# kamalmostafa/minimodem

Hardware: AMD Instinct MI355X
Metric: audio samples/sec demodulated (whole node), 1200-baud 48 kHz f32 (higher is better)
Workload: dtype f64; 1 GPU; configs[1]: Bell202 1200-baud, 48 kHz f32, batch of 1024 synthetic streams; 1024 streams x 480000 samples per GPU (BASELINE.json); streams_per_gpu=1024, total_streams=1024, input_dtype=f32, accumulate_dtype=f64

## Files before the change

minimodem_amd/__init__.py:

```python
import contextlib
import ctypes as C
import os
import subprocess

import numpy as np

from . import _lib
from ._lib import ModemArgs, RxConfig

__all__ = ["build", "rx_config", "Context", "demod_batch", "find_frame_batch",
           "LegacyPlan", "synthesize", "FRAME_DTYPE", "EPISODE_DTYPE",
           "gather_bytes", "shard_range"]

_HERE = os.path.dirname(os.path.abspath(__file__))

FRAME_DTYPE = np.dtype([("bits", "<u8"), ("start", "<u8"), ("confidence", "<f4"),
                        ("amplitude", "<f4"), ("flags", "<u4"), ("reserved", "<u4")])
EPISODE_DTYPE = np.dtype([("carrier_nsamples", "<u8"), ("first_frame", "<u4"),
                          ("nframes", "<u4"), ("confidence_total", "<f4"),
                          ("amplitude_total", "<f4"), ("end_reason", "<u4"),
                          ("b_mark", "<u4")])
SEARCH_DTYPE = np.dtype([("sample_offset", "<u8"), ("navail", "<u4"), ("try_first", "<u4"),
                         ("try_max", "<u4"), ("try_step", "<u4"), ("search_limit", "<f4"),
                         ("use_sync_string", "<u4")])
RESULT_DTYPE = np.dtype([("bits", "<u8"), ("confidence", "<f4"), ("amplitude", "<f4"),
                         ("frame_start", "<u4"), ("n_positions", "<u4")])
assert SEARCH_DTYPE.itemsize == 32 and RESULT_DTYPE.itemsize == 24
NCOUNTERS = 32
COUNTER_NAMES = {0: "iterations", 1: "batches", 2: "stages", 3: "bulk_frames", 4: "refines",
                 5: "cache_hits", 6: "positions", 7: "lattice_batches", 8: "cyc_total",
                 9: "cyc_scan", 10: "cyc_wait", 11: "cyc_confidence", 12: "cyc_bulk", 13: "w_stage", 14: "w_correlate",
                 15: "w_barrier", 16: "cyc_general", 17: "cyc_restart", 18: "cyc_scan1", 19: "cyc_scan2", 20: "cyc_replay_scan", 21: "cyc_scan_wait",
                 24: "conf_fallbacks", 25: "seg_second_looks"}


def build(force=False):
    if force and os.path.exists(_lib.LIB_PATH):
        os.unlink(_lib.LIB_PATH)
    subprocess.run(["make", "-s", "-C", os.path.join(_HERE, "csrc")], check=True)
    return _lib.LIB_PATH


def rx_config(baudmode="1200", **opts):
    lib = _lib.load()
    a = ModemArgs()
    lib.mifsk_modem_args_default(C.byref(a))
    a.baudmode = str(baudmode).encode()
    if "sync_byte" in opts:
        a.have_sync_byte = 1
    for k, v in opts.items():
        if not hasattr(a, k):
            raise TypeError("unknown modem option %r" % k)
        setattr(a, k, v)
    cfg = RxConfig()
    rc = lib.mifsk_rx_config_init(C.byref(cfg), C.byref(a))
    if rc != 0:
        raise ValueError("mifsk_rx_config_init failed: %d" % rc)
    cfg._keepalive = a
    return cfg


class Context:

    def __init__(self, device=-1):
        self._lib = _lib.load()
        h = C.c_void_p()
        rc = self._lib.mifsk_ctx_create(C.byref(h), int(device))
        if rc != 0:
            raise RuntimeError("mifsk_ctx_create failed: %d (no gfx950 HIP device? "
                               "this package has no CPU path)" % rc)
        self.handle = h

    @property
    def device_name(self):
        return self._lib.mifsk_ctx_device_name(self.handle).decode()

    def selftest_sqrt(self, nvalues, seed=1):
        counts = (C.c_uint64 * 4)()
        rc = self._lib.mifsk_selftest_sqrt(self.handle, int(seed), int(nvalues), counts)
        if rc != 0:
            raise RuntimeError("mifsk_selftest_sqrt failed: %d" % rc)
        return tuple(int(c) for c in counts)

    def selftest_rcp(self, c, x):
        c = np.ascontiguousarray(c, np.float32)
        x = np.ascontiguousarray(x, np.float32)
        assert c.shape == x.shape and c.ndim == 1
        rc_out, q = np.empty(c.shape, np.float64), np.empty(c.shape, np.float32)
        rc = self._lib.mifsk_selftest_rcp(self.handle, c.ctypes.data, x.ctypes.data, c.size,
                                          rc_out.ctypes.data, q.ctypes.data)
        if rc != 0:
            raise RuntimeError("mifsk_selftest_rcp failed: %d" % rc)
        return rc_out, q

    def selftest_mag(self, re, im, scalar=1.0):
        re = np.ascontiguousarray(re, np.float64)
        im = np.ascontiguousarray(im, np.float64)
        assert re.shape == im.shape and re.ndim == 1
        root, g = np.empty(re.shape, np.float64), np.empty(re.shape, np.float64)
        unsafe, mag = np.empty(re.shape, np.uint8), np.empty(re.shape, np.float32)
        rc = self._lib.mifsk_selftest_mag(self.handle, re.ctypes.data, im.ctypes.data, float(scalar),
                                          re.size, root.ctypes.data, g.ctypes.data,
                                          unsafe.ctypes.data, mag.ctypes.data)
        if rc != 0:
            raise RuntimeError("mifsk_selftest_mag failed: %d" % rc)
        return root, g, unsafe, mag

    def selftest_confidence(self, variant, mags, req_mask=0, req_val=0):
        mags = np.ascontiguousarray(mags, np.float32)
        assert mags.ndim == 3 and mags.shape[2] == 2
        n = mags.shape[0]
        conf, ampl = np.empty(n, np.float32), np.empty(n, np.float32)
        bits, fb = np.empty(n, np.uint64), np.empty(n, np.uint32)
        rc = self._lib.mifsk_selftest_confidence(self.handle, int(variant), mags.shape[1],
                                                 int(req_mask), int(req_val), mags.ctypes.data, n,
                                                 conf.ctypes.data, ampl.ctypes.data,
# ... 1199 lines not shown
```

minimodem_amd/csrc/mifsk_kernels.hip:

```cpp
#include <hip/hip_runtime.h>
#include <cfloat>
#include <cmath>
#include <cstdint>
#include <cstdlib>
#include <cstdio>
#include <cstring>

#include "mifsk_device.h"
#include "mifsk_devmath.h"
#include "mifsk_devlib.h"
#include "mifsk_rxloop.h"

#ifdef MIFSK_PROFILE
#define MIFSK_CLOCK() ((uint32_t)clock64())
#else
#define MIFSK_CLOCK() 0u
#endif

namespace mifsk {




__global__ __launch_bounds__(64)
// ... 143 lines not shown
	    const uint32_t v = v0 + i * blockDim.x + threadIdx.x;
	    if ( v0 + i * blockDim.x < nvec )
		buf[i] = load4_raw(x, org4 + ( v << 2 ), N);
	}
#pragma unroll
	for ( int i = 0; i < STAGE_VEC; i++ ) {
	    const uint32_t v = v0 + i * blockDim.x + threadIdx.x;
	    if ( v0 + i * blockDim.x < nvec && v < nvec )
		store4_skewed(cfg, lds->slab, slab_cap, v << 2, head, buf[i], org4 + ( v << 2 ), N);
	}
    }
}

template <bool USE_SLAB>
__device__ __forceinline__ void par_correlate( const DevCfg &cfg, const double *__restrict__ tw, StreamLds *lds,
	const float *__restrict__ x, uint32_t N, uint32_t row_org, uint32_t nq )
{
    const uint32_t n_bits = cfg.n_bits;
    const uint32_t B = cfg.bit_nsamples;
    const uint32_t nwin = nq * n_bits;
    for ( uint32_t w0 = 0; w0 < nwin; w0 += blockDim.x ) {
	const uint32_t w = w0 + threadIdx.x;
	if ( w0 + ( threadIdx.x & ~63u ) >= nwin )
	    continue;
	const bool active = w < nwin;
	const uint32_t q = active ? udiv_magic(w, n_bits, cfg.nbits_magic) : 0;
	const uint32_t k = active ? w - q * n_bits : 0;
	const uint32_t a = lds->c_pos[q] + cfg.bit_offset[k];
	double acc[4] = { 0.0, 0.0, 0.0, 0.0 };
	if ( USE_SLAB ) {
	    corr_skewed_stream(cfg, tw, lds->slab, a - row_org, threadIdx.x & 63u, acc);
	} else {
	    for ( uint32_t n = 0; n < B; n++ ) {
		const uint32_t idx = a + n;
		const float xv = ( idx < N && idx >= a ) ? x[idx] : 0.0f;
		const double xd = (double)xv;
		const double *t = tw + 4 * (size_t)n;
		acc[0] = fma(xd, t[0], acc[0]);
		acc[1] = fma(xd, t[1], acc[1]);
		acc[2] = fma(xd, t[2], acc[2]);
		acc[3] = fma(xd, t[3], acc[3]);
	    }
	}
	if ( active )
	    lds->mags[0][w] = band_mag2(acc[0], acc[1], acc[2], acc[3], cfg.magscalar);
    }
}

template <bool USE_SLAB>
__device__ __forceinline__ void scan_part( const DevCfg &cfg, const double *__restrict__ tw,
	StreamLds *lds, const StreamLds::Cmd *cmd, const float *__restrict__ x, uint32_t N,
	uint32_t slab_cap )
{
    const uint32_t nq = cmd->nq;
    const uint32_t row_org = cmd->row_org;
    if ( USE_SLAB && cmd->stage ) {
	par_stage(cfg, lds, x, N, slab_cap, row_org, cmd->stage);
	lds_barrier();
    }
    par_correlate<USE_SLAB>(cfg, tw, lds, x, N, row_org, nq);
    lds_barrier();
}

__device__ __forceinline__ void lds_barrier()
{
    __builtin_amdgcn_fence(__ATOMIC_RELEASE, "workgroup", "local");
    __builtin_amdgcn_s_barrier();
    __builtin_amdgcn_fence(__ATOMIC_ACQUIRE, "workgroup", "local");
}



template <bool USE_SLAB>
struct Master {
    const DevCfg	&cfg;
    const double	*tw;
    const float		*x;
    uint32_t		N;
    StreamLds		*lds;
    uint32_t		slab_cap;
    uint32_t		slab_lo, slab_hi;
    uint32_t		lat_batch;
    uint32_t		conf_idx;
    uint32_t		lat_first;
    uint32_t		spec, run, cold, pause;
    uint32_t		spec_floor;
    uint32_t		lane;
    bool		inflight;
    uint32_t		inflight_anchor, inflight_frames, inflight_buf;
    uint32_t		seq;
    uint32_t		lat_n, lat_anchor;
    uint32_t		hit_base = 0xFFFFFFFFu;
    bool		cnt_on = false;
    uint32_t		cyc_par = 0, cyc_conf = 0, cyc_wait = 0, cyc_scan_wait = 0;
    uint32_t		cyc_sf_load = 0, cyc_sf_corr = 0, cyc_sf_score = 0, cyc_sf_sel = 0;
    uint32_t		h_la, h_la_magic, h_nbits;
    uint64_t		h_req_mask, h_req_val;
    TwGroup		mtg[3];

    template <int NG>
    __device__ __forceinline__ void keep_groups()
    {
#pragma unroll
	for ( int gi = 0; gi < NG; gi++ )
	    mtg[gi] = tw_group_load(tw, (uint32_t)gi, lane);
    }

    __device__ __forceinline__ Master( const DevCfg &c, const double *t, const float *xs,
	    uint32_t n, StreamLds *l, uint32_t cap, uint32_t lf, uint32_t lat_round )
	: cfg(c), tw(t), x(xs), N(n), lds(l), slab_cap(cap), slab_lo(0), slab_hi(0),
	  lat_batch(lf), lane(threadIdx.x), inflight(false), inflight_anchor(0),
	  inflight_frames(0), inflight_buf(0), seq(0), lat_n(0), lat_anchor(0)
    {
	lat_first = lat_round;
	spec = lat_batch;
	run = cold = pause = 0;
	spec_floor = 2;
	h_la = keep_scalar(cfg.lock_advance);
	h_la_magic = keep_scalar(cfg.la_magic);
	h_nbits = keep_scalar(cfg.n_bits);
	h_req_mask = keep_scalar(cfg.req_mask[0]);
	h_req_val = keep_scalar(cfg.req_val[0]);
	conf_idx = lane * cfg.n_bits;
	if ( cfg.lat_grid && lat_round ) {
	    const uint32_t r = lane / lat_round, fr = lane - r * lat_round;
	    conf_idx = r * ( lat_round * ( cfg.n_bits - 1u ) + 1u ) + fr * ( cfg.n_bits - 1u );
	}
    }

    __device__ __forceinline__ void bump( uint32_t which, uint32_t by = 1u ) const
    {
	if ( cnt_on && lane == 0 )
	    (void)__hip_atomic_fetch_add(&lds->cnt[which], by, __ATOMIC_RELAXED, __HIP_MEMORY_SCOPE_WAVEFRONT);
    }

    __device__ __forceinline__ uint32_t lattice_lookup( uint32_t p ) const
    {
	if ( !lat_n || p < lat_anchor )
	    return ~0u;
	const uint32_t d = p - lat_anchor;
	const uint32_t e = udiv_magic(d, h_la, h_la_magic);
	return ( e < lat_n && e * h_la == d ) ? e : ~0u;
    }

    __device__ __forceinline__ StreamLds::Cmd *next_cmd() { return &lds->cmd[seq & 1u]; }

    __device__ __forceinline__ uint32_t lattice_frames_at( uint32_t anchor ) const
    {
	if ( anchor >= N )
	    return 0;
	const uint32_t left = udiv_magic(N - anchor - 1u, h_la, h_la_magic) + 1u;
	return left < lat_batch ? left : lat_batch;
    }

    __device__ __forceinline__ void publish_lattice( uint32_t anchor, uint32_t frames, uint32_t buf )
    {
	if ( lane == 0 ) {
	    StreamLds::Cmd *c = next_cmd();
	    c->op = frames ? CMD_LATTICE : CMD_IDLE;
	    c->anchor = anchor;
	    c->frames = frames;
	    c->buf = buf;
	}
	inflight = frames != 0;
	inflight_anchor = anchor;
	inflight_frames = frames;
	inflight_buf = buf;
	slab_lo = slab_hi = 0;
    }

    __device__ __forceinline__ void lattice_start( uint32_t anchor )
    {
	uint32_t frames = lattice_frames_at(anchor);
	if ( !frames )
	    return;
	frames = frames < lat_first ? frames : lat_first;
	frames = frames < spec ? frames : spec;
	publish_lattice(anchor, frames, 0);
	lds_barrier();
	seq++;
    }

    __device__ __forceinline__ void lattice_advance()
    {
	const uint32_t anchor = inflight_anchor, frames = inflight_frames, buf = inflight_buf;
	const uint32_t next = anchor + frames * h_la;
	uint32_t nf = lattice_frames_at(next);
	nf = nf < spec ? nf : spec;
	publish_lattice(next, nf, buf ^ 1u);
	const uint32_t t_w = MIFSK_CLOCK();
	lds_barrier();
	seq++;
	const uint32_t t_c = MIFSK_CLOCK();
	cyc_wait += t_c - t_w;
	bump(MIFSK_CNT_LATTICE_BATCHES);
	if ( lane < frames ) {
	    uint32_t fb = 0u;
	    const FrameOut fo = frame_confidence_any_staged(&lds->mags[buf][conf_idx], h_req_mask, h_req_val, h_nbits,
							    fb);
	    if ( cnt_on && fb )
		bump(MIFSK_CNT_CONF_FALLBACKS);
	    lds->c_conf[lane] = fo.conf;
	    lds->c_ampl[lane] = fo.ampl;
	    lds->c_bits[lane] = fo.bits;
	}
	lat_n = frames;
	lat_anchor = anchor;
	wave_lds_sync();
	cyc_conf += MIFSK_CLOCK() - t_c;
    }

    __device__ __forceinline__ void give_up()
    {
	if ( inflight && lane == 0 )
	    lds_poke(&lds->abort, seq);
	inflight = false;
    }

    __device__ __forceinline__ void evaluate( uint32_t nq, uint32_t kind, uint32_t lo, uint32_t hi )
    {
	bool restage = false;
	if ( USE_SLAB && ( lo < slab_lo || hi > slab_hi ) ) {
	    restage = true;
	    slab_lo = lo;
	    const uint32_t need = ( hi - lo + 7u ) & ~3u;
	    slab_hi = lo + ( ( kind == 0u && lat_batch && need < slab_cap ) ? need : slab_cap );
	    bump(MIFSK_CNT_STAGES);
	}
	StreamLds::Cmd *c = next_cmd();
	if ( lane == 0 ) {
	    c->op = CMD_SCAN;
	    c->nq = nq;
	    c->stage = restage ? slab_hi - slab_lo : 0u;
	    c->row_org = slab_lo;
	}
	if ( inflight && lane == 0 )
	    lds_poke(&lds->abort, seq);
	inflight = false;
	bump(MIFSK_CNT_BATCHES);
	bump(MIFSK_CNT_POSITIONS, nq);
	const uint32_t t_par = MIFSK_CLOCK();
	lds_barrier();
	seq++;
	cyc_scan_wait += MIFSK_CLOCK() - t_par;
	scan_part<USE_SLAB>(cfg, tw, lds, c, x, N, slab_cap);
	const uint32_t t_conf = MIFSK_CLOCK();
	cyc_par += t_conf - t_par;
	if ( lane < nq ) {
	    uint32_t fb = 0u;
	    const FrameOut f = frame_confidence_any_staged(&lds->mags[0][lane * cfg.n_bits],
						cfg.req_mask[kind], cfg.req_val[kind], cfg.n_bits, fb);
	    if ( cnt_on && fb )
		bump(MIFSK_CNT_CONF_FALLBACKS);
	    lds->c_conf[lane] = f.conf;
	    lds->c_ampl[lane] = f.ampl;
	    lds->c_bits[lane] = f.bits;
	}
	wave_lds_sync();
	cyc_conf += MIFSK_CLOCK() - t_conf;
    }

    template <int NQ>
    __device__ __forceinline__ bool solo_fine( uint32_t base, const ZigZag &zz, uint32_t first,
	    const ScanResult &c0, ScanResult &r )
    {
	static_assert(NQ >= 1 && NQ <= 12, "three table groups");
	constexpr uint32_t B = 4u * NQ;
	const uint32_t nb = cfg.n_bits;
	const uint32_t nwin = ( zz.J - 1u ) * nb;
	if ( zz.J < 2u || nwin > 128u || zz.J - 1u > 64u )
	    return false;
	const uint32_t t_sf0 = MIFSK_CLOCK();
	const uint32_t lo = base + first - zz.D * zz.step + cfg.bit_offset[0];
	const uint32_t hi = base + first + ( zz.U - 1u ) * zz.step + cfg.bit_offset[( nb - 1u ) & 63u] + B;
	const uint32_t org4 = lo;
	const bool pairs = ( zz.step & 1u ) == 0u;
	const uint32_t nvec = ( hi - org4 + 3u ) >> 2;
	if ( hi > N || hi < lo || org4 + 4u * nvec > N || nvec > 128u
		|| nvec * 16u + nwin * sizeof(float2) > sizeof(lds->mags[0]) )
	    return false;
	float *sbuf = reinterpret_cast<float *>(lds->mags[inflight ? ( inflight_buf ^ 1u ) : 0u]);
	float2 *sm = reinterpret_cast<float2 *>(sbuf + 4u * nvec);
	{
	    const bool h0 = lane < nvec, h1 = lane + 64u < nvec;
	    float4_u v0, v1;
	    if ( h0 ) v0 = *reinterpret_cast<const float4_u *>(x + org4 + 4u * lane);
	    if ( h1 ) v1 = *reinterpret_cast<const float4_u *>(x + org4 + 4u * ( lane + 64u ));
	    if ( h0 ) *reinterpret_cast<float4 *>(sbuf + 4u * lane) = make_float4(v0.x, v0.y, v0.z, v0.w);
	    if ( h1 ) *reinterpret_cast<float4 *>(sbuf + 4u * ( lane + 64u )) = make_float4(v1.x, v1.y, v1.z, v1.w);
	}
	const TwGroup (&tg)[3] = mtg;
	wave_lds_sync();
#ifdef MIFSK_PROFILE
	asm volatile("s_waitcnt vmcnt(0) lgkmcnt(0)" ::: "memory");
#endif
	const uint32_t t_sf1 = MIFSK_CLOCK();
	{
	    const uint32_t wA = lane < nwin ? lane : 0u;
	    const uint32_t wB = lane + 64u < nwin ? lane + 64u : wA;
	    const uint32_t qA = udiv_magic(wA, nb, cfg.nbits_magic), qB = udiv_magic(wB, nb, cfg.nbits_magic);
	    const bool grid = cfg.lat_grid != 0u;
	    const uint32_t kA = wA - qA * nb, kB = wB - qB * nb;
	    const uint32_t oA = grid ? kA * B : cfg.bit_offset[kA & 63u], oB = grid ? kB * B : cfg.bit_offset[kB & 63u];
	    const float *pA = sbuf + ( base + zz.at(1u + qA) + oA - org4 );
	    const float *pB = sbuf + ( base + zz.at(1u + qB) + oB - org4 );
	    double accA[4] = { 0.0, 0.0, 0.0, 0.0 }, accB[4] = { 0.0, 0.0, 0.0, 0.0 };
	    auto quad_of = [&]( const float *p, int q ) -> float4 {
		if ( pairs ) {
		    const float2 a = *reinterpret_cast<const float2 *>(p + 4 * q);
		    const float2 b = *reinterpret_cast<const float2 *>(p + 4 * q + 2);
		    return make_float4(a.x, a.y, b.x, b.y);
		}
		return make_float4(p[4 * q], p[4 * q + 1], p[4 * q + 2], p[4 * q + 3]);
	    };
	    float4 xa = quad_of(pA, 0), xb = quad_of(pB, 0);
	    dpp_settle();
#define MIFSK_SOLO2_SAMPLE(J, G, XA, XB) fma4_bcast<J>(accA, G, XA); fma4_bcast<J>(accB, G, XB);
#define MIFSK_SOLO2_QUAD(Q)									\
	    if ( (Q) < NQ ) {									\
		const float4 ca = xa, cb = xb;							\
		if ( (Q) + 1 < NQ ) {			\
		    xa = quad_of(pA, (Q) + 1 < NQ ? (Q) + 1 : 0);					\
		    xb = quad_of(pB, (Q) + 1 < NQ ? (Q) + 1 : 0);					\
		}										\
		const TwGroup &G = tg[(Q) / 4 < 3 ? (Q) / 4 : 0];					\
		MIFSK_SOLO2_SAMPLE(4 * ( (Q) % 4 ) + 0, G, ca.x, cb.x)					\
		MIFSK_SOLO2_SAMPLE(4 * ( (Q) % 4 ) + 1, G, ca.y, cb.y)					\
		MIFSK_SOLO2_SAMPLE(4 * ( (Q) % 4 ) + 2, G, ca.z, cb.z)					\
		MIFSK_SOLO2_SAMPLE(4 * ( (Q) % 4 ) + 3, G, ca.w, cb.w)					\
	    }
	    MIFSK_SOLO2_QUAD(0) MIFSK_SOLO2_QUAD(1) MIFSK_SOLO2_QUAD(2) MIFSK_SOLO2_QUAD(3)
	    MIFSK_SOLO2_QUAD(4) MIFSK_SOLO2_QUAD(5) MIFSK_SOLO2_QUAD(6) MIFSK_SOLO2_QUAD(7)
	    MIFSK_SOLO2_QUAD(8) MIFSK_SOLO2_QUAD(9) MIFSK_SOLO2_QUAD(10) MIFSK_SOLO2_QUAD(11)
#undef MIFSK_SOLO2_QUAD
#undef MIFSK_SOLO2_SAMPLE
	    if ( lane < nwin )
		sm[lane] = band_mag2(accA[0], accA[1], accA[2], accA[3], cfg.magscalar);
	    if ( lane + 64u < nwin )
		sm[lane + 64u] = band_mag2(accB[0], accB[1], accB[2], accB[3], cfg.magscalar);
	}
	wave_lds_sync();
	const uint32_t t_sf2 = MIFSK_CLOCK();
	FrameOut f;
	f.conf = 0.0f; f.ampl = 0.0f; f.bits = 0;
	if ( lane < zz.J - 1u ) {
	    uint32_t fb = 0u;
	    f = frame_confidence_any_staged(&sm[lane * nb], cfg.req_mask[0], cfg.req_val[0], nb, fb);
	    if ( cnt_on && fb )
		bump(MIFSK_CNT_CONF_FALLBACKS);
	}
	bump(MIFSK_CNT_POSITIONS, zz.J - 1u);
	const uint32_t t_sf3 = MIFSK_CLOCK();
	r = c0;
	uint32_t win = 0;
	{
	    const bool cand = lane < zz.J - 1u && f.conf == f.conf;
	    const float best = wave_max_f32(cand ? f.conf : -INFINITY);
	    if ( r.conf < best ) {
		const unsigned long long at = __ballot(cand && f.conf == best);
		win = (uint32_t)__ffsll((long long)at);
		r.conf = best;
	    }
	}
	if ( win ) {
	    r.ampl = lane_bcast(f.ampl, win - 1u);
	    const uint32_t blo = (uint32_t)__builtin_amdgcn_readlane((int)(uint32_t)f.bits, (int)( win - 1u ));
	    const uint32_t bhi = (uint32_t)__builtin_amdgcn_readlane((int)(uint32_t)( f.bits >> 32 ), (int)( win - 1u ));
	    r.bits = ( (uint64_t)bhi << 32 ) | blo;
	    r.start = zz.at(win);
	}
	cyc_sf_load += t_sf1 - t_sf0;
	cyc_sf_corr += t_sf2 - t_sf1;
	cyc_sf_score += t_sf3 - t_sf2;
	cyc_sf_sel += MIFSK_CLOCK() - t_sf3;
	return true;
    }

    __device__ __forceinline__ ScanResult scan( uint32_t base, const ZigZag &zz, uint32_t first,
	    float limit, uint32_t kind )
    {
	ScanResult r;
	r.conf = 0.0f; r.ampl = 0.0f; r.bits = 0; r.start = 0;
	hit_base = 0xFFFFFFFFu;
	if ( zz.J == 0 )
	    return r;
	const uint32_t p0 = base + first;

	{
	    const uint32_t hit = kind == 0u ? lattice_lookup(p0) : ~0u;
	    if ( hit != ~0u ) {
		const float c = lds->c_conf[hit];
		if ( c > 0.0f && c >= limit ) {
		    r.conf = c;
		    r.ampl = lds->c_ampl[hit];
		    r.bits = lds->c_bits[hit];
		    r.start = first;
		    bump(MIFSK_CNT_CACHE_HITS);
		    hit_base = base;
		    return r;
		}
	    }
	}

	uint32_t qmax = W_CAP / cfg.n_bits;
	if ( qmax > P_CAP ) qmax = P_CAP;
	bool done = false;
	for ( uint32_t c0 = 0; c0 < zz.J && !done; c0 += qmax ) {
	    const uint32_t Q = zz.J - c0 < qmax ? zz.J - c0 : qmax;
	    const uint32_t iend = c0 + Q - 1u;
	    const uint32_t lu = iend > 2u * zz.D ? iend : ( ( iend & 1u ) ? iend : iend - 1u );
	    const uint32_t ld = ( iend < 2u * zz.D ? iend : 2u * zz.D ) & ~1u;
	    const bool has_up = lu >= ( c0 > 1u ? c0 : 1u ) && lu <= iend && iend >= 1u;
	    const bool has_down = ld >= 2u && ld >= c0;
	    const uint32_t thi = has_up ? zz.at(lu) : zz.at(c0);
	    const uint32_t tlo = has_down ? zz.at(ld) : zz.at(c0);
	    if ( lane < Q )
		lds->c_pos[lane] = base + zz.at(c0 + lane);
	    lat_n = 0;
	    evaluate(Q, kind, base + tlo, base + thi + cfg.last_reach);
	    const float cl = lane < Q ? lds->c_conf[lane] : 0.0f;
	    uint32_t win = ~0u;
	    for ( uint32_t i = 0; i < Q; i++ ) {
		const float c = lane_bcast(cl, i);
		if ( r.conf < c ) {
		    r.conf = c;
		    win = i;
		    if ( r.conf >= limit ) {
			done = true;
			break;
		    }
		}
	    }
	    if ( win != ~0u ) {
		r.ampl = lds->c_ampl[win];
		r.bits = lds->c_bits[win];
		r.start = zz.at(c0 + win);
	    }
	}
	return r;
    }
};


struct WgResume : ResumeArgs {
    uint32_t		bufsize;
};

struct DemodArgs {
    const DevCfg	*cfgp;
    const double	*tw;
    mifsk_demod_io	io;
    uint32_t		slab_cap, lat_frames, lat_rounds, region_floats, region_cap, lat_mode;
    WgResume		rs;
};

template <bool USE_SLAB, int NQ, bool ST>
__device__ __forceinline__ void master_loop( const DevCfg &cfg, const double *__restrict__ tw,
	const mifsk_demod_io &io, uint32_t slab_cap, uint32_t lat_frames, uint32_t lat_round,
	uint32_t lat_mode, uint32_t base0, StreamLds *lds, const WgResume &rs )
{
    const uint32_t s = blockIdx.x;
    const float *x = io.d_samples + (size_t)s * io.stream_stride;
    uint32_t N = row_nsamples(io, s);
    const bool cut = chain_cut<ST>(rs.d_state, rs.limit, N);
    const StreamOut o = StreamOut::make(io, s);
    const uint32_t lane = threadIdx.x;
    const bool t0 = lane == 0;

    Master<USE_SLAB> ctx(cfg, tw, x, N, lds, slab_cap, lat_frames, lat_round);
    if constexpr ( NQ > 0 )
	ctx.template keep_groups<( NQ + 3 ) / 4>();
    const uint32_t h_first1 = keep_scalar(cfg.try_first[1]);
    const uint32_t h_expect = keep_scalar(cfg.expect_nsamples);
    const uint32_t h_fn = keep_scalar(cfg.frame_nsamples);
    const uint32_t h_overscan = keep_scalar(cfg.overscan);
    const float h_limit = keep_scalar(cfg.search_limit);
    const float h_thr = keep_scalar(cfg.conf_threshold);
    const uint32_t h_dshift = keep_scalar(( cfg.has_stopbits ? 1u : 0u ) + cfg.nstartbits);
    const uint64_t h_dmask = keep_scalar(cfg.n_data_bits >= 64u ? ~0ULL : ( 1ULL << cfg.n_data_bits ) - 1ULL);
    const bool h_msb = cfg.msb_first != 0u;
    const bool h_rx_sync = cfg.do_rx_sync != 0u;
    const uint64_t h_sync_byte = keep_scalar(cfg.sync_byte);
    const uint32_t h_try_max0 = keep_scalar(cfg.try_max[0]), h_try_max1 = keep_scalar(cfg.try_max[1]);
    const uint32_t h_try_step0 = keep_scalar(cfg.try_step[0]), h_try_step1 = keep_scalar(cfg.try_step[1]);
    const uint32_t h_first0 = keep_scalar(cfg.try_first[0]);
    if ( lat_mode == LAT_LINEAR )
	ctx.spec_floor = lat_round;
    ctx.cnt_on = io.d_counters != nullptr;

    bool carrier = false;
    float confidence_total = 0.0f, amplitude_total = 0.0f;
    uint32_t nframes_decoded = 0;
    uint64_t carrier_nsamples = 0;
    uint32_t noconfidence = 0;
    uint32_t advance = 0;
    float track_amplitude = 0.0f, peak_confidence = 0.0f;

    uint32_t base = base0 < N ? base0 : N;
    uint32_t n_out_frames = 0, n_out_bytes = 0, n_out_eps = 0, ep_first = 0;
    uint32_t ep_b_mark = 0;
    uint32_t status = 0;

    const bool stateful = ST && rs.d_state != nullptr;
    const bool last_slab = !stateful || rs.final != 0u || ( rs.limit != 0u && !cut );
    uint64_t origin = 0;
    uint32_t frame_base = 0;
    bool resumable = true;
    uint32_t rp = base;
    if constexpr ( ST ) {
	if ( stateful ) {
	    if ( rs.d_origin )
		origin = rs.d_origin[s];
	    const mifsk_stream_state st = rs.d_state[s];
	    if ( st.flags & MIFSK_STATE_FINISHED ) {
		resumable = false;
		if ( rs.append == 0u )
		    status |= st.status & MIFSK_STREAM_ABORTED;
	    } else if ( st.flags & MIFSK_STATE_STARTED ) {
		if ( st.base < origin || st.base - origin > (uint64_t)N || st.rp < st.base ) {
		    status |= MIFSK_STREAM_ABORTED;
		    resumable = false;
		} else {
		    auto u32 = []( uint32_t v ) { return (uint32_t)__builtin_amdgcn_readfirstlane((int)v); };
		    auto f32 = [&]( float v ) { return __uint_as_float(u32(__float_as_uint(v))); };
		    base = u32((uint32_t)( st.base - origin ));
		    rp = base + u32((uint32_t)( st.rp - st.base ));
		    advance = u32(st.advance);
		    carrier = ( u32(st.flags) & MIFSK_STATE_CARRIER ) != 0u;
		    carrier_nsamples = ( (uint64_t)u32((uint32_t)( st.carrier_nsamples >> 32 )) << 32 )
				     | u32((uint32_t)st.carrier_nsamples);
		    confidence_total = f32(st.confidence_total);
		    amplitude_total = f32(st.amplitude_total);
		    nframes_decoded = u32(st.nframes_decoded);
		    noconfidence = u32(st.noconfidence);
		    track_amplitude = f32(st.track_amplitude);
		    peak_confidence = f32(st.peak_confidence);
		    ep_first = u32(st.ep_first);
		    ep_b_mark = u32(st.ep_b_mark);
		    frame_base = u32((uint32_t)st.nframes_total);
		    if ( rs.append ) {
			n_out_frames = frame_base;
			n_out_bytes = u32(st.nbytes_total);
			n_out_eps = u32(st.nepisodes_total);
			status = u32(st.status);
			frame_base = 0u;
		    }
		}
	    }
	}
    }
    const uint32_t bufsize = ST ? rs.bufsize : 0u, half = bufsize / 2u;
    const uint32_t N_lat = last_slab ? N : ( N > bufsize ? N - bufsize : 0u );
    bool paused = false;

    uint32_t cyc_bulk = 0, cyc_general = 0, cyc_restart = 0, cyc_s1 = 0, cyc_s2 = 0, cyc_dpp = 0;
    const uint32_t t_start = MIFSK_CLOCK();
#ifdef MIFSK_PROFILE
    const uint32_t t_wall0 = (uint32_t)wall_clock64();
#endif

    const ZigZag zc0(cfg, 0u), zc1(cfg, 1u), zf0(cfg, 2u), zf1(cfg, 3u);

    for (;;) {
	if ( ST && !resumable )
	    break;
	bool fwd = false;
	ScanResult fwd_sr;
	fwd_sr.conf = 0.0f; fwd_sr.ampl = 0.0f; fwd_sr.bits = 0; fwd_sr.start = 0;
	if ( carrier && advance && ( ST ? ( base <= N_lat && advance <= N_lat - base && advance <= rp - base )
					: advance <= N - base ) ) {
	    const uint32_t t_bulk = MIFSK_CLOCK();
	    const uint32_t first = h_first1;
	    const uint32_t nb = base + advance;
	    const uint32_t p = nb + first;
	    const uint32_t e0 = ctx.lattice_lookup(p);
	    bool progressed = false, broke = false;
	    if ( e0 != ~0u ) {
		uint32_t K = ctx.lat_n - e0;
		const uint32_t fn = h_fn;
		const uint32_t la = ctx.h_la;
		const uint32_t room = N_lat - nb >= h_expect
				    ? udiv_magic(N_lat - nb - h_expect, la, ctx.h_la_magic) + 1u : 0u;
		K = K < room ? K : room;
		const bool have = lane < K;
		const float cv = have ? lds->c_conf[e0 + lane] : 0.0f;
		const float av = have ? lds->c_ampl[e0 + lane] : 0.0f;
		const uint32_t t_dpp = MIFSK_CLOCK();
		float xt = ( track_amplitude + av ) / 2.0f;
		float xpk = peak_confidence < cv ? cv : peak_confidence;
		float xsc = confidence_total + cv;
		float xsa = amplitude_total + av;
		float my_t = track_amplitude, my_pk = peak_confidence;
		float my_sc = confidence_total, my_sa = amplitude_total;
		replay_scan_asm(xt, xpk, xsc, xsa, my_t, my_pk, my_sc, my_sa, cv, av, K, o.eps != nullptr);
		cyc_dpp += MIFSK_CLOCK() - t_dpp;
		const float t = xt, pk = xpk, sc = xsc, sa = xsa;
		const bool ok = have
		    && cv > 0.0f && cv >= h_limit
		    && !( cv < my_pk * 0.75f )
		    && !( av < my_t * 0.25f )
		    && !( cv <= h_thr );
		const unsigned long long bad = __ballot(have && !ok);
		const uint32_t n = bad ? (uint32_t)__ffsll((long long)bad) - 1u : K;
		float track, peak, ctot, atot;
		if ( n == K ) {
		    track = lane_bcast(t, K - 1u);
		    peak = lane_bcast(pk, K - 1u);
		    ctot = lane_bcast(sc, K - 1u);
		    atot = lane_bcast(sa, K - 1u);
		} else {
		    track = lane_bcast(my_t, n);
		    peak = lane_bcast(my_pk, n);
		    ctot = lane_bcast(my_sc, n);
		    atot = lane_bcast(my_sa, n);
		}
		ctx.run += n;
		if ( NQ == 0 && bad != 0ULL && cfg.try_step[1] > 1u )
		    ctx.give_up();
		if ( n < K ) {
		    ctx.spec = ctx.run < ctx.spec_floor ? ctx.spec_floor
			     : ( ctx.run < ctx.lat_batch ? ctx.run : ctx.lat_batch );
		    ctx.cold = ctx.run ? 0u : ctx.cold + 1u;
		    ctx.run = 0;
		} else if ( e0 + K == ctx.lat_n ) {
		    ctx.spec = 2u * ctx.spec < ctx.lat_batch ? 2u * ctx.spec : ctx.lat_batch;
		}
		if ( n ) {
		    const bool mine = lane < n;
		    uint64_t db = 0;
		    bool suppressed = false;
		    if ( mine ) {
			db = ( lds->c_bits[e0 + lane] >> h_dshift ) & h_dmask;
			if ( h_msb )
			    db = bit_reverse(db, cfg.n_data_bits);
			suppressed = h_rx_sync && db == h_sync_byte;
		    }
		    const unsigned long long keep = __ballot(mine && !suppressed);

		    if ( mine ) {
			const uint32_t fi = n_out_frames + lane;
// ... 76 lines not shown
		if ( advance > rp - base )
		    break;
		base += advance;
		advance = 0;
	    }
	    if ( rp - base < half )
		rp += N - rp < half ? N - rp : half;
	    const uint32_t nvalid = rp - base;
	    if ( nvalid == 0 || nvalid < cfg.expect_nsamples )
		break;
	} else {
	    if ( advance ) {
		if ( advance > N - base )
		    break;
		base += advance;
		advance = 0;
	    }
	    const uint32_t avail = N - base;
	    if ( avail == 0 || avail < h_expect )
		break;
	}
	ctx.bump(MIFSK_CNT_ITERATIONS);
	const uint32_t t_gen = MIFSK_CLOCK();

	const uint32_t ci = carrier ? 1u : 0u;
	const uint32_t try_max = carrier ? h_try_max1 : h_try_max0;
	const uint32_t try_step = carrier ? h_try_step1 : h_try_step0;
	const uint32_t try_first = carrier ? h_first1 : h_first0;

	const uint32_t t_s1 = MIFSK_CLOCK();
	ScanResult sr;
	if ( fwd ) {
	    sr = fwd_sr;
	    ctx.hit_base = base;
	    ctx.bump(MIFSK_CNT_CACHE_HITS);
	} else {
	    sr = ctx.scan(base, carrier ? zc1 : zc0, try_first, h_limit, carrier ? 0u : 1u);
	}
	cyc_s1 += MIFSK_CLOCK() - t_s1;
	float confidence = sr.conf;
	float amplitude = sr.ampl;
	uint64_t bits = sr.bits;
	uint32_t frame_start = sr.start;

	bool refine = false;
	if ( confidence < peak_confidence * 0.75f ) {
	    refine = true;
	    peak_confidence = 0.0f;
	}
	if ( amplitude < track_amplitude * 0.25f )
	    confidence = 0.0f;

	if ( confidence <= h_thr ) {
	    if ( ++noconfidence > 20u ) {
		if ( carrier ) {
		    store_episode(o, t0, n_out_eps, carrier_nsamples, ep_first, nframes_decoded,
				  confidence_total, amplitude_total, 1u, cfg.b_mark);
		    n_out_eps++;
		    carrier = false;
		    carrier_nsamples = 0;
		    confidence_total = 0.0f;
		    amplitude_total = 0.0f;
		    nframes_decoded = 0;
		    track_amplitude = 0.0f;
		    if ( cfg.rx_one )
			break;
		}
	    }
	    advance = try_max;
	    continue;
	}

	carrier_nsamples += h_fn;
	uint32_t flags = 0;
	if ( carrier ) {
	    carrier_nsamples += frame_start;
	    carrier_nsamples -= h_overscan;
	} else {
	    carrier = true;
	    refine = true;
	    flags |= MIFSK_FRAME_ACQUIRE;
	    ep_first = frame_base + n_out_frames;
	    ep_b_mark = cfg.b_mark;
	}

	if ( refine && confidence < INFINITY && try_step > 1u ) {
	    const uint32_t t_s2 = MIFSK_CLOCK();
	    ScanResult s2;
	    bool alone = false;
	    if constexpr ( NQ > 0 ) {
		if ( ci && ctx.hit_base == base )
		    alone = ctx.template solo_fine<NQ>(base, zf1, try_first, sr, s2);
	    }
	    if ( !alone )
		s2 = ctx.scan(base, ci ? zf1 : zf0, try_first, INFINITY, 0u);
	    cyc_s2 += MIFSK_CLOCK() - t_s2;
	    flags |= MIFSK_FRAME_REFINED;
	    ctx.bump(MIFSK_CNT_REFINES);
	    if ( s2.conf > confidence ) {
		bits = s2.bits;
		amplitude = s2.ampl;
		frame_start = s2.start;
	    }
	}

	advance = frame_start + h_fn - h_overscan;

	if ( ctx.lat_batch && advance <= N - base ) {
	    const uint32_t p = base + advance + h_first1;
	    const bool cached = ctx.lattice_lookup(p) != ~0u;
	    const uint32_t t_ls = MIFSK_CLOCK();
	    if ( ctx.pause ) {
		ctx.pause--;
	    } else if ( !cached && !( ctx.inflight && ctx.inflight_anchor == p ) ) {
		ctx.give_up();
		if ( ctx.cold >= 4u ) {
		    ctx.cold = 0;
		    ctx.pause = 32;
		} else {
		    ctx.lattice_start(p);
		}
	    }
	    cyc_restart += MIFSK_CLOCK() - t_ls;
	}

	track_amplitude = ( track_amplitude + amplitude ) / 2.0f;
	if ( peak_confidence < confidence )
	    peak_confidence = confidence;
	confidence_total += confidence;
	amplitude_total += amplitude;
	nframes_decoded++;
	noconfidence = 0;

	bits = ( bits >> h_dshift ) & h_dmask;
	if ( h_msb )
	    bits = bit_reverse(bits, cfg.n_data_bits);
	const bool suppressed = h_rx_sync && bits == h_sync_byte;
	if ( suppressed )
	    flags |= MIFSK_FRAME_SYNC;

	if ( t0 ) {

	    if ( n_out_frames < o.fcap ) {
		if ( o.bits )
		    o.bits[n_out_frames] = bits;
		if ( o.frames ) {
		    mifsk_frame f;
		    f.bits = bits;
		    f.start = origin + (uint64_t)base + frame_start;
		    f.confidence = confidence;
		    f.amplitude = amplitude;
		    f.flags = flags;
		    f.reserved = 0;
		    o.frames[n_out_frames] = f;
		}
	    }
	    if ( !suppressed && o.bytes && n_out_bytes < o.fcap )
		o.bytes[n_out_bytes] = (uint8_t)( bits & 0xFFu );
	}
	n_out_frames++;
	if ( !suppressed )
	    n_out_bytes++;

	cyc_general += MIFSK_CLOCK() - t_gen;
    }


    if constexpr ( ST ) {
	if ( stateful && t0 && !( status & MIFSK_STREAM_ABORTED ) && resumable ) {
	    mifsk_stream_state st;
	    st.base = origin + base;
	    st.rp = origin + rp;
	    st.carrier_nsamples = carrier_nsamples;
	    st.nframes_total = (uint64_t)frame_base + n_out_frames;
	    st.advance = advance;
	    st.flags = MIFSK_STATE_STARTED | ( carrier ? MIFSK_STATE_CARRIER : 0u )
		     | ( paused ? 0u : MIFSK_STATE_FINISHED );
	    st.confidence_total = confidence_total;
	    st.amplitude_total = amplitude_total;
	    st.nframes_decoded = nframes_decoded;
	    st.noconfidence = noconfidence;
	    st.track_amplitude = track_amplitude;
	    st.peak_confidence = peak_confidence;
	    const bool was_started = ( rs.d_state[s].flags & MIFSK_STATE_STARTED ) != 0u;
	    st.carrier_band = was_started ? rs.d_state[s].carrier_band : -1;
	    st.first_band = was_started ? rs.d_state[s].first_band : -1;
	    st.b_mark = cfg.b_mark;
	    st.ep_b_mark = ep_b_mark;
	    st.ep_first = ep_first;
	    const uint32_t b0 = rs.append ? 0u : rs.d_state[s].nbytes_total, e0 = rs.append ? 0u : rs.d_state[s].nepisodes_total;
	    st.nbytes_total = b0 + n_out_bytes;
	    st.nepisodes_total = e0 + n_out_eps;
	    st.status = rs.d_state[s].status | status;
	    rs.d_state[s] = st;
	} else if ( stateful && t0 && ( status & MIFSK_STREAM_ABORTED ) ) {
	    mifsk_stream_state st = rs.d_state[s];
	    st.flags |= MIFSK_STATE_STARTED | MIFSK_STATE_FINISHED;
	    st.status |= MIFSK_STREAM_ABORTED;
	    rs.d_state[s] = st;
	}
    }
    if ( carrier && !( ST && ( paused || !resumable ) ) ) {
	store_episode(o, t0, n_out_eps, carrier_nsamples, ep_first, nframes_decoded,
		      confidence_total, amplitude_total, 2u, cfg.b_mark);
	n_out_eps++;
    }
    if ( t0 && !( ST && rs.append != 0u && !resumable && status == 0u ) ) {
	if ( n_out_frames > o.fcap && ( o.bits || o.frames || o.bytes ) )
	    status |= MIFSK_STREAM_FRAMES_TRUNCATED;
	if ( n_out_eps > o.ecap && o.eps )
	    status |= MIFSK_STREAM_EPISODES_TRUNCATED;
	const KernArgs<DemodArgs>::ptr a = KernArgs<DemodArgs>::here();
	if ( a->io.d_nframes ) a->io.d_nframes[s] = n_out_frames;
	if ( a->io.d_nbytes ) a->io.d_nbytes[s] = n_out_bytes;
	if ( a->io.d_nepisodes ) a->io.d_nepisodes[s] = n_out_eps;
	if ( a->io.d_status ) a->io.d_status[s] = status;
	if ( a->io.d_counters ) {
	    uint64_t *c = a->io.d_counters + (size_t)s * MIFSK_NCOUNTERS;
	    for ( int i = 0; i < MIFSK_NCOUNTERS; i++ )
		c[i] = lds->cnt[i];
	    c[MIFSK_CNT_CYC_TOTAL] = MIFSK_CLOCK() - t_start;
	    c[MIFSK_CNT_CYC_PARALLEL] = ctx.cyc_par;
	    c[MIFSK_CNT_CYC_WAIT] = ctx.cyc_wait;
	    c[MIFSK_CNT_CYC_CONFIDENCE] = ctx.cyc_conf;
	    c[MIFSK_CNT_CYC_BULK] = cyc_bulk;
	    c[16] = cyc_general;
	    c[17] = cyc_restart | ( (uint64_t)ctx.cyc_sf_load << 32 );
	    c[18] = cyc_s1 | ( (uint64_t)ctx.cyc_sf_corr << 32 );
	    c[19] = cyc_s2 | ( (uint64_t)ctx.cyc_sf_score << 32 );
	    c[20] = cyc_dpp;
	    c[21] = ctx.cyc_scan_wait | ( (uint64_t)ctx.cyc_sf_sel << 32 );
#ifdef MIFSK_PROFILE
	    c[23] = ( wall_clock64() & 0xFFFFFFFFull ) | ( (uint64_t)t_wall0 << 32 );
	    c[22] = (uint64_t)( __builtin_amdgcn_s_getreg(( 3 << 11 ) | 20) & 15 ) << 32;
#endif
	}
    }
    if ( t0 )
	ctx.next_cmd()->op = CMD_EXIT;
    lds_barrier();
}


struct WorkerHot {
    uint32_t	n_bits, B, la;
    bool	grid;
    float	magscalar;
    uint32_t	buf, total, anchor0;
};

template <int NQ>
__device__ __forceinline__ void worker_lattice_linear( const WorkerHot &h, const double *__restrict__ tw,
	StreamLds *lds, const float *__restrict__ x, uint32_t N,
	uint32_t region_floats, uint32_t lat_frames, uint32_t wkr, uint32_t done, uint32_t win_base,
	uint32_t rel_lane, uint32_t safe_limit,
	float4 (&pbuf)[STAGE_VEC], uint32_t &pref_org4, uint32_t (&wcyc)[6], const TwGroup (&tgr)[3] )
{
    uint32_t lane = threadIdx.x & 63u;
    asm volatile("" : "+v"(lane));
    const uint32_t n_bits = h.n_bits, B = h.B;
    if ( h.grid )
	rel_lane = ( wkr * 64u + lane ) * B;
    const uint32_t buf = h.buf;
    float *region = lds->slab + (size_t)wkr * region_floats;
    const uint32_t total = h.total;
    {
	const uint32_t t_in = MIFSK_CLOCK();
	const uint32_t frames = total - done < lat_frames ? total - done : lat_frames;
	const uint32_t anchor = h.anchor0 + done * h.la;
	const uint32_t nwin = h.grid ? frames * ( n_bits - 1u ) + 1u : frames * n_bits;
	const uint32_t w = wkr * 64u + lane;
	if ( wkr * 64u >= nwin ) {
	    pref_org4 = 0xFFFFFFFFu;
	    return;
	}
	const bool active = w < nwin;
	const uint32_t last = nwin - wkr * 64u > 64u ? 63u : nwin - wkr * 64u - 1u;
	const uint32_t a1 = anchor + rel_lane;
	const uint32_t lo = (uint32_t)__builtin_amdgcn_readfirstlane((int)a1);
	const uint32_t hi = (uint32_t)__builtin_amdgcn_readlane((int)a1, (int)last) + B;
	const uint32_t a = active ? a1 : lo;
	const uint32_t nvec = ( hi - lo + 3 ) >> 2;

	constexpr uint32_t kRoundFloats = 64u * STAGE_VEC * 4u;
	if ( pref_org4 != lo ) {
	    const bool ok = lo <= safe_limit - kRoundFloats;
	    const float *pb = x + ( ok ? lo : 0u ) + ( lane << 2 );
#pragma unroll
	    for ( int i = 0; i < STAGE_VEC; i++ ) {
		const float4_u sv = *reinterpret_cast<const float4_u *>(pb + i * 256);
		pbuf[i] = make_float4(sv.x, sv.y, sv.z, sv.w);
	    }
	}
#ifdef MIFSK_PROFILE
	asm volatile("s_waitcnt vmcnt(0)" ::: "memory");
#endif
	const uint32_t t_a = MIFSK_CLOCK();
	float *lane_base = region + ( lane << 2 );
	const uint32_t nvec_lane = nvec > lane ? nvec - lane : 0u;
	const uint32_t elast = lo + kRoundFloats;
	if ( elast <= N && elast >= lo && region_floats >= kRoundFloats ) {
#pragma unroll
	    for ( int i = 0; i < STAGE_VEC; i++ )
		*reinterpret_cast<float4 *>(lane_base + i * 256) = pbuf[i];
	} else if ( elast <= N && elast >= lo ) {
#pragma unroll
	    for ( int i = 0; i < STAGE_VEC; i++ )
		if ( (uint32_t)( i * 64 ) < nvec_lane )
		    *reinterpret_cast<float4 *>(lane_base + i * 256) = pbuf[i];
	} else {
#pragma unroll
	    for ( int i = 0; i < STAGE_VEC; i++ ) {
		const uint32_t e = lo + ( ( i * 64 + lane ) << 2 );
		float4 sv;
		sv.x = ( e < N ) ? x[e] : 0.0f;
		sv.y = ( e + 1 < N && e + 1 > e ) ? x[e + 1] : 0.0f;
		sv.z = ( e + 2 < N && e + 2 > e ) ? x[e + 2] : 0.0f;
		sv.w = ( e + 3 < N && e + 3 > e ) ? x[e + 3] : 0.0f;
		if ( (uint32_t)( i * 64 ) < nvec_lane )
		    *reinterpret_cast<float4 *>(lane_base + i * 256) = sv;
	    }
	}
	const uint32_t t_b = MIFSK_CLOCK();
	{
	    const uint32_t nlo = lo + lat_frames * h.la;
	    const bool ok = nlo >= lo && nlo <= safe_limit - kRoundFloats;
	    const float *pb = x + ( ok ? nlo : 0u ) + ( lane << 2 );
#pragma unroll
	    for ( int i = 0; i < STAGE_VEC; i++ ) {
		const float4_u sv = *reinterpret_cast<const float4_u *>(pb + i * 256);
		pbuf[i] = make_float4(sv.x, sv.y, sv.z, sv.w);
	    }
	    pref_org4 = ok ? nlo : 0xFFFFFFFFu;
	}
	const uint32_t t_c = MIFSK_CLOCK();
	wave_lds_sync();
	const uint32_t t_mid = MIFSK_CLOCK();
	wcyc[3] += t_a - t_in;
	wcyc[4] += t_b - t_a;
	wcyc[5] += t_c - t_b;

	double mr = 0.0, mi = 0.0, sr = 0.0, si = 0.0;
	if constexpr ( NQ > 0 ) {
	    double acc[4] = { 0.0, 0.0, 0.0, 0.0 };
	    corr_lds_fixed_halves<NQ>(tgr, region + ( a - lo ), acc);
	    mr = acc[0]; mi = acc[1]; sr = acc[2]; si = acc[3];
	} else {
	    double acc[4] = { 0.0, 0.0, 0.0, 0.0 };
	    corr_lds_stream_lean(tw, region + ( a - lo ), B >> 2, lane, acc);
	    mr = acc[0]; mi = acc[1]; sr = acc[2]; si = acc[3];
	}
	if ( active )
	    lds->mags[buf][win_base + w] = band_mag2(mr, mi, sr, si, h.magscalar);
	wave_lds_sync();
	const uint32_t t_out = MIFSK_CLOCK();
	wcyc[0] += t_mid - t_in;
	wcyc[1] += t_out - t_mid;
    }
}


__device__ __forceinline__ void worker_lattice_direct( const DevCfg &cfg, const double *__restrict__ tw,
	StreamLds *lds, const StreamLds::Cmd *cmd, const float *__restrict__ x, uint32_t N,
	uint32_t lat_frames, uint32_t wkr, uint32_t done, uint32_t win_base, uint32_t (&wcyc)[6] )
{
    const uint32_t t_in = MIFSK_CLOCK();
    const uint32_t lane = threadIdx.x & 63u;
    const uint32_t n_bits = cfg.n_bits, B = cfg.bit_nsamples;
    const uint32_t total = cmd->frames;
    const uint32_t frames = total - done < lat_frames ? total - done : lat_frames;
    const uint32_t anchor = cmd->anchor + done * cfg.lock_advance;
    const uint32_t nwin = cfg.lat_grid ? frames * ( n_bits - 1u ) + 1u : frames * n_bits;
    const uint32_t w = wkr * 64u + lane;
    if ( wkr * 64u >= nwin )
	return;
    const bool active = w < nwin;
    const uint32_t wc = active ? w : wkr * 64u;
    uint32_t a;
    if ( cfg.lat_grid ) {
	a = anchor + wc * B;
    } else {
	const uint32_t f = udiv_magic(wc, n_bits, cfg.nbits_magic);
	a = anchor + f * cfg.lock_advance + cfg.bit_offset[( wc - f * n_bits ) & 63u];
    }
    const uint32_t Bpad = ( B + 15u ) & ~15u;
    double acc[4] = { 0.0, 0.0, 0.0, 0.0 };
    if ( __all(a + Bpad <= N && a + Bpad >= a) ) {
	corr_global_stream(tw, x + a, B, lane, acc);
    } else {
	for ( uint32_t n = 0; n < B; n++ ) {
	    const uint32_t idx = a + n;
	    const double xd = (double)( ( idx < N && idx >= a ) ? x[idx] : 0.0f );
	    const double *t = tw + 4 * (size_t)n;
	    acc[0] = fma(xd, t[0], acc[0]);
	    acc[1] = fma(xd, t[1], acc[1]);
	    acc[2] = fma(xd, t[2], acc[2]);
	    acc[3] = fma(xd, t[3], acc[3]);
	}
    }
    if ( active )
	lds->mags[cmd->buf][win_base + w] = band_mag2(acc[0], acc[1], acc[2], acc[3], cfg.magscalar);
// ... 251 lines not shown
```

Measured before the change: 1480 billion samples/s.

## Replace serial scan winner loop with wave ballot/max and vectorize tail staging

Replaces the per-lane serial broadcast loop that picks the first candidate exceeding the confidence limit with a ballot to find the stop lane plus a wave-wide max reduction. The edge-case staging path now reuses prefetched float4 data, or loads clamped float4 vectors, instead of four scalar global loads per lane. It also removes the lat_first cap on the first lattice batch and adds profile-only timing counters. Tie-breaking and NaN handling in the winner selection change subtly, and removing the first-batch cap alters the speculative lattice ramp.

Measured after the change: 1484 billion samples/s (median of 5 runs). No clear change (+0.3%).

```diff
diff --git a/minimodem_amd/__init__.py b/minimodem_amd/__init__.py
--- a/minimodem_amd/__init__.py
+++ b/minimodem_amd/__init__.py
@@ -31,7 +31,8 @@
                  5: "cache_hits", 6: "positions", 7: "lattice_batches", 8: "cyc_total",
                  9: "cyc_scan", 10: "cyc_wait", 11: "cyc_confidence", 12: "cyc_bulk", 13: "w_stage", 14: "w_correlate",
                  15: "w_barrier", 16: "cyc_general", 17: "cyc_restart", 18: "cyc_scan1", 19: "cyc_scan2", 20: "cyc_replay_scan", 21: "cyc_scan_wait",
-                 24: "conf_fallbacks", 25: "seg_second_looks"}
+                 24: "conf_fallbacks", 25: "seg_second_looks",
+                 26: "cyc_to_acquire", 27: "cyc_acquire_fine", 28: "cyc_ramp", 29: "cyc_last_wait", 30: "cyc_after_last"}
 
 
 def build(force=False):
diff --git a/minimodem_amd/csrc/mifsk_kernels.hip b/minimodem_amd/csrc/mifsk_kernels.hip
--- a/minimodem_amd/csrc/mifsk_kernels.hip
+++ b/minimodem_amd/csrc/mifsk_kernels.hip
@@ -249,7 +249,6 @@
     uint32_t		slab_lo, slab_hi;
     uint32_t		lat_batch;
     uint32_t		conf_idx;
-    uint32_t		lat_first;
     uint32_t		spec, run, cold, pause;
     uint32_t		spec_floor;
     uint32_t		lane;
@@ -261,6 +260,12 @@
     bool		cnt_on = false;
     uint32_t		cyc_par = 0, cyc_conf = 0, cyc_wait = 0, cyc_scan_wait = 0;
     uint32_t		cyc_sf_load = 0, cyc_sf_corr = 0, cyc_sf_score = 0, cyc_sf_sel = 0;
+#ifdef MIFSK_PROFILE
+    uint32_t		t_ramp0 = 0, t_ramp1 = 0, last_wait = 0, t_last_batch = 0;
+    bool		ramp_open = false, ramp_done = false;
+    uint32_t		t_origin = 0, scans_seen = 0;
+    uint32_t		sa0 = 0, sa1 = 0, sa2 = 0, sa3 = 0, sa4 = 0, sb1 = 0, sb2 = 0, sb3 = 0, sb4 = 0;
+#endif
     uint32_t		h_la, h_la_magic, h_nbits;
     uint64_t		h_req_mask, h_req_val;
     TwGroup		mtg[3];
@@ -279,7 +284,6 @@
 	  lat_batch(lf), lane(threadIdx.x), inflight(false), inflight_anchor(0),
 	  inflight_frames(0), inflight_buf(0), seq(0), lat_n(0), lat_anchor(0)
     {
-	lat_first = lat_round;
 	spec = lat_batch;
 	run = cold = pause = 0;
 	spec_floor = 2;
@@ -341,8 +345,13 @@
 	uint32_t frames = lattice_frames_at(anchor);
 	if ( !frames )
 	    return;
-	frames = frames < lat_first ? frames : lat_first;
 	frames = frames < spec ? frames : spec;
+#ifdef MIFSK_PROFILE
+	if ( !ramp_open ) {
+	    ramp_open = true;
+	    t_ramp0 = MIFSK_CLOCK();
+	}
+#endif
 	publish_lattice(anchor, frames, 0);
 	lds_barrier();
 	seq++;
@@ -375,6 +384,14 @@
 	lat_anchor = anchor;
 	wave_lds_sync();
 	cyc_conf += MIFSK_CLOCK() - t_c;
+#ifdef MIFSK_PROFILE
+	last_wait = t_c - t_w;
+	t_last_batch = MIFSK_CLOCK();
+	if ( !ramp_done && frames == lat_batch ) {
+	    ramp_done = true;
+	    t_ramp1 = t_last_batch;
+	}
+#endif
     }
 
     __device__ __forceinline__ void give_up()
@@ -410,7 +427,18 @@
 	lds_barrier();
 	seq++;
 	cyc_scan_wait += MIFSK_CLOCK() - t_par;
+#ifdef MIFSK_PROFILE
+	const uint32_t t_pub = MIFSK_CLOCK();
+	if ( USE_SLAB && c->stage ) {
+	    par_stage(cfg, lds, x, N, slab_cap, c->row_org, c->stage);
+	    lds_barrier();
+	}
+	const uint32_t t_staged = MIFSK_CLOCK();
+	par_correlate<USE_SLAB>(cfg, tw, lds, x, N, c->row_org, c->nq);
+	lds_barrier();
+#else
 	scan_part<USE_SLAB>(cfg, tw, lds, c, x, N, slab_cap);
+#endif
 	const uint32_t t_conf = MIFSK_CLOCK();
 	cyc_par += t_conf - t_par;
 	if ( lane < nq ) {
@@ -425,6 +453,21 @@
 	}
 	wave_lds_sync();
 	cyc_conf += MIFSK_CLOCK() - t_conf;
+#ifdef MIFSK_PROFILE
+	if ( scans_seen == 0u ) {
+	    sa0 = t_par - t_origin;
+	    sa1 = t_pub - t_par;
+	    sa2 = t_staged - t_pub;
+	    sa3 = t_conf - t_staged;
+	    sa4 = MIFSK_CLOCK() - t_conf;
+	} else if ( scans_seen == 1u ) {
+	    sb1 = t_pub - t_par;
+	    sb2 = t_staged - t_pub;
+	    sb3 = t_conf - t_staged;
+	    sb4 = MIFSK_CLOCK() - t_conf;
+	}
+	scans_seen++;
+#endif
     }
 
     template <int NQ>
@@ -586,17 +629,15 @@
 	    lat_n = 0;
 	    evaluate(Q, kind, base + tlo, base + thi + cfg.last_reach);
 	    const float cl = lane < Q ? lds->c_conf[lane] : 0.0f;
+	    const unsigned long long stop = __ballot(lane < Q && cl >= limit && cl > r.conf);
+	    const uint32_t last = stop ? (uint32_t)__ffsll((long long)stop) - 1u : Q - 1u;
+	    done = stop != 0ULL;
+	    const bool cand = lane <= last && cl == cl;
+	    const float best = wave_max_f32(cand ? cl : -INFINITY);
 	    uint32_t win = ~0u;
-	    for ( uint32_t i = 0; i < Q; i++ ) {
-		const float c = lane_bcast(cl, i);
-		if ( r.conf < c ) {
-		    r.conf = c;
-		    win = i;
-		    if ( r.conf >= limit ) {
-			done = true;
-			break;
-		    }
-		}
+	    if ( r.conf < best ) {
+		win = (uint32_t)__ffsll((long long)__ballot(cand && cl == best)) - 1u;
+		r.conf = best;
 	    }
 	    if ( win != ~0u ) {
 		r.ampl = lds->c_ampl[win];
@@ -721,8 +762,13 @@
     bool paused = false;
 
     uint32_t cyc_bulk = 0, cyc_general = 0, cyc_restart = 0, cyc_s1 = 0, cyc_s2 = 0, cyc_dpp = 0;
+#ifdef MIFSK_PROFILE
+    uint32_t cyc_to_acquire = 0, cyc_acq_fine = 0;
+    bool acquired_once = false;
+#endif
     const uint32_t t_start = MIFSK_CLOCK();
 #ifdef MIFSK_PROFILE
+    ctx.t_origin = t_start;
     const uint32_t t_wall0 = (uint32_t)wall_clock64();
 #endif
 
@@ -965,6 +1011,10 @@
 	    flags |= MIFSK_FRAME_ACQUIRE;
 	    ep_first = frame_base + n_out_frames;
 	    ep_b_mark = cfg.b_mark;
+#ifdef MIFSK_PROFILE
+	    if ( !acquired_once )
+		cyc_to_acquire = MIFSK_CLOCK() - t_start;
+#endif
 	}
 
 	if ( refine && confidence < INFINITY && try_step > 1u ) {
@@ -978,6 +1028,10 @@
 	    if ( !alone )
 		s2 = ctx.scan(base, ci ? zf1 : zf0, try_first, INFINITY, 0u);
 	    cyc_s2 += MIFSK_CLOCK() - t_s2;
+#ifdef MIFSK_PROFILE
+	    if ( !ci && !acquired_once )
+		cyc_acq_fine = MIFSK_CLOCK() - t_s2;
+#endif
 	    flags |= MIFSK_FRAME_REFINED;
 	    ctx.bump(MIFSK_CNT_REFINES);
 	    if ( s2.conf > confidence ) {
@@ -987,6 +1041,9 @@
 	    }
 	}
 
+#ifdef MIFSK_PROFILE
+	acquired_once = true;
+#endif
 	advance = frame_start + h_fn - h_overscan;
 
 	if ( ctx.lat_batch && advance <= N - base ) {
@@ -1116,6 +1173,15 @@
 #ifdef MIFSK_PROFILE
 	    c[23] = ( wall_clock64() & 0xFFFFFFFFull ) | ( (uint64_t)t_wall0 << 32 );
 	    c[22] = (uint64_t)( __builtin_amdgcn_s_getreg(( 3 << 11 ) | 20) & 15 ) << 32;
+	    c[26] = cyc_to_acquire | ( (uint64_t)ctx.sa0 << 32 );
+	    c[27] = cyc_acq_fine | ( (uint64_t)ctx.sa1 << 32 );
+	    c[28] = ( ctx.ramp_done ? ctx.t_ramp1 - ctx.t_ramp0 : 0u ) | ( (uint64_t)ctx.sa2 << 32 );
+	    c[29] = ctx.last_wait | ( (uint64_t)ctx.sa3 << 32 );
+	    c[30] = ( ctx.t_last_batch ? MIFSK_CLOCK() - ctx.t_last_batch : 0u ) | ( (uint64_t)ctx.sa4 << 32 );
+	    {
+		auto q12 = []( uint32_t v ) -> uint64_t { return ( v >> 6 ) < 4095u ? ( v >> 6 ) : 4095u; };
+		c[31] = q12(ctx.sb1) | ( q12(ctx.sb2) << 12 ) | ( q12(ctx.sb3) << 24 ) | ( q12(ctx.sb4) << 36 );
+	    }
 #endif
 	}
     }
@@ -1192,14 +1258,30 @@
 		if ( (uint32_t)( i * 64 ) < nvec_lane )
 		    *reinterpret_cast<float4 *>(lane_base + i * 256) = pbuf[i];
 	} else {
+	    const bool whole = lo <= safe_limit - kRoundFloats;
+	    const uint32_t top = safe_limit - 4u;
+	    if ( !whole ) {
+#pragma unroll
+		for ( int i = 0; i < STAGE_VEC; i++ ) {
+		    const uint32_t e = lo + ( ( i * 64 + lane ) << 2 );
+		    const float4_u sv = *reinterpret_cast<const float4_u *>(x + ( e < top ? e : top ));
+		    pbuf[i] = make_float4(sv.x, sv.y, sv.z, sv.w);
+		}
+	    }
 #pragma unroll
 	    for ( int i = 0; i < STAGE_VEC; i++ ) {
 		const uint32_t e = lo + ( ( i * 64 + lane ) << 2 );
+		const uint32_t d = ( whole || e < top ) ? 0u : e - top;
+		const float4 p = pbuf[i];
 		float4 sv;
-		sv.x = ( e < N ) ? x[e] : 0.0f;
-		sv.y = ( e + 1 < N && e + 1 > e ) ? x[e + 1] : 0.0f;
-		sv.z = ( e + 2 < N && e + 2 > e ) ? x[e + 2] : 0.0f;
-		sv.w = ( e + 3 < N && e + 3 > e ) ? x[e + 3] : 0.0f;
+		sv.x = d == 0u ? p.x : d == 1u ? p.y : d == 2u ? p.z : d == 3u ? p.w : 0.0f;
+		sv.y = d == 0u ? p.y : d == 1u ? p.z : d == 2u ? p.w : 0.0f;
+		sv.z = d == 0u ? p.z : d == 1u ? p.w : 0.0f;
+		sv.w = d == 0u ? p.w : 0.0f;
+		sv.x = ( e < N ) ? sv.x : 0.0f;
+		sv.y = ( e + 1 < N && e + 1 > e ) ? sv.y : 0.0f;
+		sv.z = ( e + 2 < N && e + 2 > e ) ? sv.z : 0.0f;
+		sv.w = ( e + 3 < N && e + 3 > e ) ? sv.w : 0.0f;
 		if ( (uint32_t)( i * 64 ) < nvec_lane )
 		    *reinterpret_cast<float4 *>(lane_base + i * 256) = sv;
 	    }
```
